# dibbelab/gficf

Measured on AMD Instinct MI355X. Metric: jaccard_edges_per_sec, higher is better.
Workload: dtype int32; 1 GPU; north-star point: 100000 cells x k=30 per GPU; N_total=100000; 8 independent data sets per step, windowed kNN (W=100) with permuted ids; per data set: ingest + edge kernel, one library call, device-resident, one stream, in order (no overlap between data sets or steps); rows taken to hold distinct ids: no duplicate scan in the ingest, the edge kernel's hash-set build reports a repeated id (deferred; cells_total=100000, k=30, partition=cell blocks x1

## Files before the change

### gficf_amd/csrc/jaccard.hip

```cpp
#include <atomic>
#include <cmath>
#include <cstdlib>
#include <cstring>
#include <thread>
#include <type_traits>
#include <vector>

#include "common.h"
#include "halo_map.h"

#include "jaccard_shared.h"
#include "jaccard_ingest.h"
#include "jaccard_edges_general.h"
#include "jaccard_edges_pipe.h"
#include "jaccard_edges_bits.h"
#include "jaccard_sorted.h"
#include "jaccard_direct.h"

namespace {


static_assert(std::is_same<decltype(&k_jaccard_edges<32, false, false, OUT_RMAT, false>), EdgeKernFn>::value &&
              std::is_same<decltype(&k_jaccard_edges<64, false, true, OUT_U16, true>), EdgeKernFn>::value &&
              std::is_same<decltype(&k_jaccard_edges_pipe<32, false, true, OUT_RMAT, true, false, true>), EdgeKernFn>::value &&
// ... 174 lines not shown
      table[(row0 + rr) * pitch + j] = v;
    }
    if (pitch == DUAL_PITCH && compact && kpad == 64) {
      const int lane = threadIdx.x & 63, wave = threadIdx.x >> 6;
      for (int rr = wave; rr < rows_here; rr += 4) {
        const uint32_t* in = s_pk + rr * wpr;
        s_ids[wave][lane] = lane < k ? packed_id(in, lane, bits, wpr, mask) : 0u;
        __builtin_amdgcn_fence(__ATOMIC_ACQ_REL, "wavefront");
        planar_row_build(s_ids[wave], k, ((in[fl_w] >> fl_b) & 1u) != 0u, s_prow[wave], lane);
        if (lane < 32) table[(row0 + rr) * pitch + 32 + lane] = s_prow[wave][lane];
        __builtin_amdgcn_fence(__ATOMIC_ACQ_REL, "wavefront");
      }
    }
    __syncthreads();
  }
}

template <typename T>
int launch_ingest(gficf_ctx* ctx, const T* d_idx, int64_t n_rows, int k, int64_t ld, int64_t N_total,
                  uint32_t* table, int zero_ok = 0) {
  if (sorted_fmt(k)) return launch_ingest_sorted<T>(ctx, d_idx, n_rows, k, ld, N_total, table, zero_ok);
  const TableFmt f = table_fmt(N_total, k);
  const int64_t cap = (int64_t)ctx->num_cus * 8;
  const int64_t tiles2 = gficf_ceil_div(n_rows, INGEST2_ROWS);
  const unsigned grid2 = (unsigned)(tiles2 < cap ? tiles2 : cap);
  const int64_t tiles = gficf_ceil_div(n_rows, INGEST_ROWS);
  const unsigned grid = (unsigned)(tiles < cap ? tiles : cap);
  static const bool use_reg = getenv("GFICF_JACCARD_INGEST_REG") != nullptr;
  const bool scan = !(ctx->jaccard_assume_distinct && zero_ok == 0);
#define LAUNCH_INGEST_REG(KP, CM)                                                                                          \
  do {                                                                                                                     \
    if (use_reg)                                                                                                           \
      hipLaunchKernelGGL((k_ingest_reg<T, KP, CM>), dim3(grid2), dim3(INGEST2_ROWS), 0, ctx->stream, d_idx, n_rows, k, ld, N_total, \
                         table, ctx->d_status, zero_ok);                                                                   \
    else if (scan)                                                                                                         \
      hipLaunchKernelGGL((k_ingest_tile<T, KP, CM>), dim3(grid), dim3(256), 0, ctx->stream, d_idx, n_rows, k, ld, N_total,  \
                         table, ctx->d_status, zero_ok, gficf_halo_map{});                                                 \
    else                                                                                                                   \
      hipLaunchKernelGGL((k_ingest_tile<T, KP, CM, false, false>), dim3(grid), dim3(256), 0, ctx->stream, d_idx, n_rows, k, ld, N_total, \
                         table, ctx->d_status, zero_ok, gficf_halo_map{});                                                 \
  } while (0)
#define LAUNCH_INGEST(KP, CM)                                                                                   \
  hipLaunchKernelGGL((k_ingest<T, KP, CM>), dim3(grid), dim3(256), 0, ctx->stream, d_idx, n_rows, k, ld, N_total, \
                     table, ctx->d_status, zero_ok, scan ? 1 : 0)
  switch (f.kpad) {
    case 16: LAUNCH_INGEST_REG(16, false); break;
    case 32: if (f.compact) LAUNCH_INGEST_REG(32, true); else LAUNCH_INGEST_REG(32, false); break;
    case 64:
      if (f.dual) {
        if (scan)
          hipLaunchKernelGGL((k_ingest_tile<T, 64, true, false, true, true>), dim3(grid), dim3(256), 0, ctx->stream, d_idx, n_rows, k, ld, N_total,
                             table, ctx->d_status, zero_ok, gficf_halo_map{});
        else
          hipLaunchKernelGGL((k_ingest_tile<T, 64, true, false, false, true>), dim3(grid), dim3(256), 0, ctx->stream, d_idx, n_rows, k, ld, N_total,
                             table, ctx->d_status, zero_ok, gficf_halo_map{});
      } else if (f.compact) LAUNCH_INGEST_REG(64, true); else LAUNCH_INGEST_REG(64, false);
      break;
    case 128: if (f.compact) LAUNCH_INGEST(128, true); else LAUNCH_INGEST(128, false); break;
    default: if (f.compact) LAUNCH_INGEST(256, true); else LAUNCH_INGEST(256, false); break;
  }
#undef LAUNCH_INGEST
#undef LAUNCH_INGEST_REG
  GFICF_HIP_CHECK(hipGetLastError());
  return GFICF_OK;
}

template <typename K>
int edge_blocks_per_cu(K kernel, int threads, size_t lds_bytes, std::atomic<int>& cache, int* out) {
  int v = cache.load(std::memory_order_relaxed);
  if (v == 0) {
    int nb = 0;
    GFICF_HIP_CHECK(hipOccupancyMaxActiveBlocksPerMultiprocessor(&nb, kernel, threads, lds_bytes));
    v = nb > 8 ? 8 : nb > 0 ? nb : 1;
    if (const char* e = getenv("GFICF_JACCARD_BLOCKS_PER_CU")) {
      const int t = atoi(e);
      if (t > 0) v = t;
    }
    cache.store(v, std::memory_order_relaxed);
  }
  *out = v;
  return GFICF_OK;
}

template <int KPAD, bool BIG, bool CMP, int OUT, bool MAP>
int launch_edges_m(gficf_ctx* ctx, const uint32_t* table, int64_t N, int k, int64_t cb, int64_t ce, EdgeOut o) {
  using C = JCfg<KPAD, CMP>;
  static std::atomic<int> bpc_general{0}, bpc_pipe{0}, bpc_pipe_nob16{0};
  constexpr size_t lds_bytes = edges_lds_bytes<KPAD, CMP>();
  int blocks_per_cu = 1;
  static const bool no_pipe = getenv("GFICF_JACCARD_NO_PIPE") != nullptr;
  if constexpr (C::EPL == 1 && C::SPQ <= 4) {
    if (!no_pipe) {
      const bool nob16 = CMP && N < 65536;
      int rc;
      if constexpr (!MAP) {
        if (o.dup_status != nullptr) {
          static std::atomic<int> bpc_nf{0}, bpc_nf_nob16{0};
          if (nob16) rc = edge_blocks_per_cu(k_jaccard_edges_pipe<KPAD, BIG, CMP, OUT, !CMP, false, true>, C::WAVES * 64, lds_bytes, bpc_nf_nob16, &blocks_per_cu);
          else rc = edge_blocks_per_cu(k_jaccard_edges_pipe<KPAD, BIG, CMP, OUT, true, false, true>, C::WAVES * 64, lds_bytes, bpc_nf, &blocks_per_cu);
          if (rc) return rc;
          const int64_t cap_n = (int64_t)ctx->num_cus * blocks_per_cu;
          const int64_t need_n = gficf_ceil_div(gficf_ceil_div(ce - cb, 4), C::WAVES);
          unsigned grid_n = (unsigned)(need_n < cap_n ? need_n : cap_n);
          if (o.xcd && grid_n > 8) grid_n = (grid_n + 7u) & ~7u;
          if (nob16)
            hipLaunchKernelGGL((k_jaccard_edges_pipe<KPAD, BIG, CMP, OUT, !CMP, false, true>), dim3(grid_n), dim3(C::WAVES * 64), lds_bytes, ctx->stream,
                               table, N, k, cb, ce, o);
          else
            hipLaunchKernelGGL((k_jaccard_edges_pipe<KPAD, BIG, CMP, OUT, true, false, true>), dim3(grid_n), dim3(C::WAVES * 64), lds_bytes, ctx->stream,
                               table, N, k, cb, ce, o);
          GFICF_HIP_CHECK(hipGetLastError());
          return GFICF_OK;
        }
      }
      if (nob16) rc = edge_blocks_per_cu(k_jaccard_edges_pipe<KPAD, BIG, CMP, OUT, !CMP, MAP>, C::WAVES * 64, lds_bytes, bpc_pipe_nob16, &blocks_per_cu);
      else rc = edge_blocks_per_cu(k_jaccard_edges_pipe<KPAD, BIG, CMP, OUT, true, MAP>, C::WAVES * 64, lds_bytes, bpc_pipe, &blocks_per_cu);
      if (rc) return rc;
      const int64_t cap = (int64_t)ctx->num_cus * blocks_per_cu;
      const int64_t need4 = gficf_ceil_div(gficf_ceil_div(ce - cb, 4), C::WAVES);
      unsigned grid4 = (unsigned)(need4 < cap ? need4 : cap);
      if (o.xcd && grid4 > 8) grid4 = (grid4 + 7u) & ~7u;
      if (nob16)
        hipLaunchKernelGGL((k_jaccard_edges_pipe<KPAD, BIG, CMP, OUT, !CMP, MAP>), dim3(grid4), dim3(C::WAVES * 64), lds_bytes, ctx->stream,
                           table, N, k, cb, ce, o);
      else
        hipLaunchKernelGGL((k_jaccard_edges_pipe<KPAD, BIG, CMP, OUT, true, MAP>), dim3(grid4), dim3(C::WAVES * 64), lds_bytes, ctx->stream, table,
                           N, k, cb, ce, o);
      GFICF_HIP_CHECK(hipGetLastError());
      return GFICF_OK;
    }
  }
  const int rc = edge_blocks_per_cu(k_jaccard_edges<KPAD, BIG, CMP, OUT, MAP>, C::WAVES * 64, lds_bytes, bpc_general, &blocks_per_cu);
  if (rc) return rc;
  const int64_t blocks_needed = gficf_ceil_div(ce - cb, C::WAVES);
  const int64_t cap = (int64_t)ctx->num_cus * blocks_per_cu;
  unsigned grid = (unsigned)(blocks_needed < cap ? blocks_needed : cap);
  if (o.xcd && grid > 8) grid = (grid + 7u) & ~7u;
  hipLaunchKernelGGL((k_jaccard_edges<KPAD, BIG, CMP, OUT, MAP>), dim3(grid), dim3(C::WAVES * 64), lds_bytes, ctx->stream, table,
                     N, k, cb, ce, o);
  GFICF_HIP_CHECK(hipGetLastError());
  return GFICF_OK;
}

template <int KPAD, bool BIG, bool CMP, int OUT>
int launch_edges_o(gficf_ctx* ctx, const uint32_t* table, int64_t N, int k, int64_t cb, int64_t ce, EdgeOut o) {
  if constexpr (OUT != OUT_U16) {
    if (o.l2g) return launch_edges_m<KPAD, BIG, CMP, OUT, true>(ctx, table, N, k, cb, ce, o);
  }
  return launch_edges_m<KPAD, BIG, CMP, OUT, false>(ctx, table, N, k, cb, ce, o);
}

template <int KPAD, bool BIG, bool CMP>
int launch_edges_t(gficf_ctx* ctx, const uint32_t* table, int64_t N, int k, int64_t cb, int64_t ce, EdgeOut o) {
  if (o.u16) return launch_edges_o<KPAD, BIG, CMP, OUT_U16>(ctx, table, N, k, cb, ce, o);
  if (o.u) return launch_edges_o<KPAD, BIG, CMP, OUT_RMAT_U>(ctx, table, N, k, cb, ce, o);
  return launch_edges_o<KPAD, BIG, CMP, OUT_RMAT>(ctx, table, N, k, cb, ce, o);
}

template <int NST, int OUT, bool MAP>
int launch_bits_m(gficf_ctx* ctx, const uint32_t* table, int64_t N, int k, int64_t cb, int64_t ce, EdgeOut o) {
  static std::atomic<int> bpc{0};
  static std::atomic<bool> attr_set[64];
  if (!attr_set[ctx->device & 63]) {
    GFICF_HIP_CHECK(hipFuncSetAttribute((const void*)k_jaccard_edges_bits<NST, OUT, MAP>, hipFuncAttributeMaxDynamicSharedMemorySize, (int)BITS_LDS_BYTES));
    attr_set[ctx->device & 63] = true;
  }
  int blocks_per_cu = 1;
  const int rc = edge_blocks_per_cu(k_jaccard_edges_bits<NST, OUT, MAP>, BITS_WAVES * 64, BITS_LDS_BYTES, bpc, &blocks_per_cu);
  if (rc) return rc;
  const int64_t need = gficf_ceil_div(ce - cb, BITS_WAVES);
  const int64_t cap = (int64_t)ctx->num_cus * blocks_per_cu;
  unsigned grid = (unsigned)(need < cap ? need : cap);
  if (o.xcd && grid > 8) grid = (grid + 7u) & ~7u;
  hipLaunchKernelGGL((k_jaccard_edges_bits<NST, OUT, MAP>), dim3(grid), dim3(BITS_WAVES * 64), BITS_LDS_BYTES, ctx->stream, table, N, k, cb, ce, o);
  GFICF_HIP_CHECK(hipGetLastError());
  return GFICF_OK;
}

template <int NST>
int launch_bits(gficf_ctx* ctx, const uint32_t* table, int64_t N, int k, int64_t cb, int64_t ce, EdgeOut o) {
  if (o.u16) return launch_bits_m<NST, OUT_U16, false>(ctx, table, N, k, cb, ce, o);
  if (o.u) return o.l2g ? launch_bits_m<NST, OUT_RMAT_U, true>(ctx, table, N, k, cb, ce, o) : launch_bits_m<NST, OUT_RMAT_U, false>(ctx, table, N, k, cb, ce, o);
  return o.l2g ? launch_bits_m<NST, OUT_RMAT, true>(ctx, table, N, k, cb, ce, o) : launch_bits_m<NST, OUT_RMAT, false>(ctx, table, N, k, cb, ce, o);
}

template <int KPAD>
int launch_edges(gficf_ctx* ctx, const uint32_t* table, int64_t N, int k, int64_t cb, int64_t ce, EdgeOut o) {
  if constexpr (KPAD == 64) {
    if (table_fmt(N, k).dual) {
      const int nst = (k + 7) / 8;
      return nst <= 5 ? launch_bits<5>(ctx, table, N, k, cb, ce, o) : nst == 6 ? launch_bits<6>(ctx, table, N, k, cb, ce, o)
                                                                                : launch_bits<7>(ctx, table, N, k, cb, ce, o);
    }
  }
  static const bool force_big = getenv("GFICF_JACCARD_FORCE_BIG") != nullptr;
  const bool big = force_big || N >= (1ll << 24) || N * (int64_t)KPAD * 4 >= (1ll << 32);
  if (KPAD >= 32 && table_fmt(N, k).compact)
    return launch_edges_t<KPAD, false, KPAD >= 32>(ctx, table, N, k, cb, ce, o);
  return big ? launch_edges_t<KPAD, true, false>(ctx, table, N, k, cb, ce, o)
             : launch_edges_t<KPAD, false, false>(ctx, table, N, k, cb, ce, o);
}

int launch_edges_k(gficf_ctx* ctx, const uint32_t* t, int64_t N, int k, int64_t cb, int64_t ce, EdgeOut o) {
  if (sorted_fmt(k)) return launch_edges_sorted(ctx, t, N, k, cb, ce, o);
// ... 684 lines not shown
```

### gficf_amd/csrc/jaccard_edges_pipe.h

```cpp

#pragma once

#include "jaccard_shared.h"

namespace {

template <int KPAD, bool BIG, bool CMP, int OUT, bool B16 = true, bool MAP = false, bool NOFLAG = false>
__global__ __launch_bounds__(jc_threads<KPAD>) void k_jaccard_edges_pipe(
    const uint32_t* __restrict__ table, int64_t N, int k, int64_t cell_begin, int64_t cell_end, EdgeOut o) {
  using C = JCfg<KPAD, CMP>;
  using F = CFmt<KPAD>;
  static_assert(C::EPL == 1 && C::SPQ <= 4, "one batch of gathers per cell");
  static_assert(!(BIG && CMP), "compact rows hold 17-bit ids");
  using off_t = typename std::conditional<BIG, uint64_t, uint32_t>::type;
  constexpr int NST = C::SPQ;
  extern __shared__ unsigned char smem[];
  constexpr uint32_t HBYTES = C::NB * 8;
  constexpr uint32_t SETS = 1;
  constexpr uint32_t WBYTES = SETS * HBYTES;
  uint32_t(*const s_rows)[2][KPAD] = reinterpret_cast<uint32_t(*)[2][KPAD]>(smem + C::WAVES * WBYTES);
  double* const s_lut = reinterpret_cast<double*>(smem + C::WAVES * WBYTES + C::WAVES * 2 * KPAD * 4);
  constexpr uint32_t STAGE_OFF = C::WAVES * WBYTES + C::WAVES * 2 * KPAD * 4 + (GFICF_JACCARD_MAX_K + 1) * 8;
  constexpr uint32_t STAGE_WAVE = 4 * 64 * 8;
  constexpr uint32_t DUPF_OFF = edges_dupflag_off<KPAD, CMP>();

  const int tid = threadIdx.x, lane = tid & 63;
  const int wave = __builtin_amdgcn_readfirstlane(tid >> 6);
  unsigned char* const hbase = smem + wave * WBYTES;
  for (int u = tid; u <= k; u += C::WAVES * 64) s_lut[u] = (double)u / (2.0 * (double)k - (double)u);
  for (int b = lane; b < (int)(SETS * C::NB); b += 64) reinterpret_cast<uint2*>(hbase)[b] = make_uint2(EMPTY, EMPTY);
  for (int t = lane; t < 4 * 64; t += 64) reinterpret_cast<uint2*>(smem + STAGE_OFF + (uint32_t)wave * STAGE_WAVE)[t] = make_uint2(0u, 0u);
  if (lane == 0) *reinterpret_cast<uint32_t*>(smem + DUPF_OFF + (uint32_t)wave * 4u) = 0u;
  __syncthreads();

  const uint32_t wave_off = lds_address(smem) + (uint32_t)(tid >> 6) * WBYTES;
  uint32_t bmask_v = (uint32_t)(C::NB - 1) << 3, bit16_v = 0x10000u;
  asm volatile("" : "+v"(bmask_v), "+v"(bit16_v));
  uint32_t* const ovlist = s_rows[wave][0];
  const char* const tbytes = reinterpret_cast<const char*>(table);
  const int grow = lane / C::LPR, gl = lane % C::LPR;
  const uint32_t gcol = (uint32_t)gl * 16u;
  const unsigned long long lt_mask = (1ull << lane) - 1ull;
  const int64_t nwaves = (int64_t)gridDim.x * C::WAVES;
  constexpr uint32_t ROWB = C::ROWB;
  constexpr int ROWW = ROWB / 4;
  const int hi_abs = F::HIW + (gl >> 2);
  const int hi_l = lane - gl + (hi_abs >> 2), hi_c = hi_abs & 3;
  const bool tail = gl >= F::KC / 8;
  const int slot_c = lane < C::NSLOT ? lane : C::NSLOT - 1;
  const bool slot_ok = lane < C::NSLOT;

  const int64_t first = cell_begin + 4 * ((int64_t)xcd_block(blockIdx.x, gridDim.x, o.xcd) * C::WAVES + wave);
  if (first >= cell_end) return;
  const int64_t last_cell = cell_end - 1;
  const int64_t quad_step = 4 * nwaves - 3;
  const uint32_t stage_w = lds_address(smem) + STAGE_OFF + (uint32_t)(tid >> 6) * STAGE_WAVE;
  int qc0, qc1;
  uint32_t qra0, qra1;
  {
    const int e0 = 2 * lane, e1 = e0 + 1;
    qc0 = (e0 >= k) + (e0 >= 2 * k) + (e0 >= 3 * k);
    qc1 = (e1 >= k) + (e1 >= 2 * k) + (e1 >= 3 * k);
    int j0 = e0 - qc0 * k, j1 = e1 - qc1 * k;
    j0 = j0 < 63 ? j0 : 63;
    j1 = j1 < 63 ? j1 : 63;
    qra0 = stage_w + (uint32_t)(qc0 * 64 + j0) * 8u;
    qra1 = stage_w + (uint32_t)(qc1 * 64 + j1) * 8u;
  }

  struct OwnRaw { uint32_t v, hw, last; };
  auto load_own = [&](int64_t row, OwnRaw& r) {
    const uint32_t* const rw = table + row * ROWW;
    if (!CMP) {
      r.v = rw[slot_c];
      r.hw = 0; r.last = 0;
    } else {
      r.last = rw[ROWW - 1];
      r.v = reinterpret_cast<const uint16_t*>(rw)[slot_c];
      r.hw = (KPAD == 32) ? 0u : rw[F::HIW + (slot_c >> 5)];
    }
  };
  auto decode_own = [&](const OwnRaw& r) -> uint32_t {
    uint32_t x;
    if (!CMP) x = r.v;
    else if (B16) x = r.v | ((((KPAD == 32 ? r.last : r.hw) >> (lane & 31)) & 1u) << 16) | (NOFLAG ? 0u : (r.last & ROW_DUP_FLAG));
    else x = r.v | (NOFLAG ? 0u : (r.last & ROW_DUP_FLAG));
    return slot_ok ? x : 0u;
  };
  auto true_id = [&](uint32_t keyraw) -> uint32_t {
    const uint32_t x = keyraw & ID_MASK;
    return CMP ? (unscramble16(x & 0xFFFFu) | (x & 0x10000u)) : x;
  };
  auto issue_gathers = [&](uint32_t asafe, uint4 (&bv)[NST]) {
#pragma unroll
    for (int st = 0; st < NST; ++st) {
      const uint32_t dst = (uint32_t)__shfl((int)asafe, st * C::RPS + grow);
      const off_t off = (off_t)(dst - 1) * ROWB + gcol;
      bv[st] = *reinterpret_cast<const uint4*>(tbytes + off);
    }
  };
  auto piece_words = [&](const uint4& bv, uint32_t (&wd)[4], uint32_t& hb) -> uint32_t {
    hb = 0;
    if (B16) {
      uint32_t hw;
      if (KPAD == 32) hw = (uint32_t)__builtin_amdgcn_update_dpp(0, (int)bv.w, 0xFF, 0xf, 0xf, false);
      else {
        hw = 0;
        { const uint32_t v = (uint32_t)__shfl((int)bv.z, hi_l); hw = hi_c == 2 ? v : hw; }
        { const uint32_t v = (uint32_t)__shfl((int)bv.w, hi_l); hw = hi_c == 3 ? v : hw; }
      }
      hb = (hw >> ((gl & 3) * 8)) & 0xFFu;
    }
    wd[0] = bv.x; wd[1] = bv.y; wd[2] = bv.z; wd[3] = bv.w;
    if (tail) {
      hb &= (1u << (F::KC % 8)) - 1u;
#pragma unroll
      for (int c = (F::KC % 8) / 2; c < 4; ++c) wd[c] = 0u;
    }
    return (gl == C::LPR - 1) ? bv.w : 0u;
  };

  auto process = [&](uint32_t araw, const uint4 (&bv)[NST], int& u_out) -> bool {
    const uint32_t a = araw & ID_MASK;
    bool slow = NOFLAG ? false : __ballot((araw & ROW_DUP_FLAG) != 0) != 0ull;
    int myslot = -1, nov = 0;
    bool dup_here = false;
    {
      bool over = false;
      if (a != 0) {
        const uint32_t key = a;
        const uint32_t bo = (CMP ? (key & ((uint32_t)(C::NB - 1) << 3)) : bucket_off<KPAD, BIG>(key)) + (uint32_t)wave * WBYTES;
        uint32_t old = atomicCAS(reinterpret_cast<uint32_t*>(smem + bo), EMPTY, key);
        if (old == EMPTY) myslot = (int)bo;
        else {
          dup_here |= old == key;
          old = atomicCAS(reinterpret_cast<uint32_t*>(smem + bo + 4), EMPTY, key);
          if (old == EMPTY) myslot = (int)bo + 4;
          else { dup_here |= old == key; over = true; }
        }
      }
      const unsigned long long om = __ballot(over);
      if (om) {
        if (over) ovlist[nov + __popcll(om & lt_mask)] = a;
        nov += __popcll(om);
        if (nov > 1) {
          wave_lds_fence();
          dup_here |= ovlist_repeats(ovlist, nov);
        }
      }
    }
    wave_lds_fence();
    uint32_t dupflags = 0;
    int myu = 0;
#pragma unroll
    for (int st = 0; st < NST; ++st) {
      int c;
      if (!CMP) {
        uint32_t miss = 0;
        uint32_t id[4] = {bv[st].x & ID_MASK, bv[st].y, bv[st].z, bv[st].w};
        if (!NOFLAG) dupflags |= bv[st].x;
        uint2 h[4];
#pragma unroll
        for (int t = 0; t < 4; ++t) h[t] = lds_read_b64(bucket_off<KPAD, BIG>(id[t]) | wave_off);
#pragma unroll
        for (int t = 0; t < 4; t += 2) {
          const uint32_t m0 = min3u_one(h[t].x ^ id[t], h[t].y ^ id[t]);
          const uint32_t m1 = min3u_one(h[t + 1].x ^ id[t + 1], h[t + 1].y ^ id[t + 1]);
          miss += m0 + m1;
        }
        c = 4 - (int)miss;
        if (nov) {
          for (int t = 0; t < nov; ++t) {
            const uint32_t ov = ovlist[t];
#pragma unroll
            for (int tt = 0; tt < 4; ++tt) c += (id[tt] == ov);
          }
        }
      } else {
        uint32_t wd[4], hb;
        const uint32_t fw = piece_words(bv[st], wd, hb);
        if (!NOFLAG) dupflags |= fw;
        c = probe_compact_piece<B16>(wd, hb, bmask_v, bit16_v, wave_off);
        if (nov) {
          for (int t = 0; t < nov; ++t) {
            const uint32_t ov = ovlist[t];
#pragma unroll
            for (int tt = 0; tt < 8; ++tt) c += (piece_key(wd, hb, tt) == ov);
          }
        }
      }
      const int rowcnt = group_sum<C::LPR>(c);
      const int v = __shfl(rowcnt, (lane % C::RPS) * C::LPR);
      myu = (lane / C::RPS == st) ? v : myu;
    }
    if (dup_here) *reinterpret_cast<uint32_t*>(smem + DUPF_OFF + (uint32_t)wave * 4u) = 1u;
    slow |= __ballot(dup_here || (!NOFLAG && (dupflags & ROW_DUP_FLAG) != 0)) != 0ull;
    if (myslot >= 0) *reinterpret_cast<uint32_t*>(smem + myslot) = EMPTY;
    wave_lds_fence();
    u_out = a != 0 ? myu : 0;
    return slow;
  };

  OwnRaw raw;
  load_own(first, raw);
  uint32_t araw_cur = decode_own(raw);
  uint4 bv_cur[NST];
  uint32_t id_cur = true_id(araw_cur);
  uint32_t gid_cur = MAP ? (uint32_t)o.l2g[(id_cur != 0 ? id_cur : (uint32_t)(first + 1)) - 1] : 0u;
  issue_gathers(id_cur != 0 ? id_cur : (uint32_t)(first + 1), bv_cur);
  {
    const int64_t i1 = first + 1;
    load_own(i1 < cell_end ? i1 : last_cell, raw);
  }
  bool any_slow = false;
  int64_t prev_i = first;
  uint32_t prev_a = 0;
  int prev_u = 0;

  typedef uint32_t v2u __attribute__((ext_vector_type(2)));
  typedef uint32_t v4u __attribute__((ext_vector_type(4)));
  typedef double v2d __attribute__((ext_vector_type(2)));
#ifndef GFICF_EDGE_STORE_AUX
#define GFICF_EDGE_STORE_AUX 2
#endif
  constexpr int EDGE_STORE_AUX = GFICF_EDGE_STORE_AUX;
  auto park_prev = [&](int c) {
    reinterpret_cast<uint2*>(smem + STAGE_OFF + (uint32_t)wave * STAGE_WAVE)[c * 64 + lane] = make_uint2(prev_a, (uint32_t)prev_u);
  };
  auto store_quad = [&](int64_t qfirst, int ncells) {
    wave_lds_fence();
    const uint2 p0 = lds_read_b64(qra0), p1 = lds_read_b64(qra1);
    const int64_t pb = (qfirst - cell_begin) * (int64_t)k;
    const int nedges = ncells * k;
    if (OUT != OUT_U16) {
      const uint32_t c1st = (uint32_t)(qfirst + 1) + o.src_off;
      const bool pos0 = p0.y > 0, pos1 = p1.y > 0;
      const v2d vs = {pos0 ? (double)(c1st + (uint32_t)qc0) : 0.0, pos1 ? (double)(c1st + (uint32_t)qc1) : 0.0};
      const v2d vd = {pos0 ? (double)p0.x : 0.0, pos1 ? (double)p1.x : 0.0};
      const v2d vw = {s_lut[p0.y], s_lut[p1.y]};
      const auto rs = __builtin_amdgcn_make_buffer_rsrc(o.src + pb, 0, nedges * 8, 0x00020000);
      const auto rd = __builtin_amdgcn_make_buffer_rsrc(o.dst + pb, 0, nedges * 8, 0x00020000);
      const auto rw = __builtin_amdgcn_make_buffer_rsrc(o.w + pb, 0, nedges * 8, 0x00020000);
      __builtin_amdgcn_raw_buffer_store_b128(__builtin_bit_cast(v4u, vs), rs, lane * 16, 0, EDGE_STORE_AUX);
      __builtin_amdgcn_raw_buffer_store_b128(__builtin_bit_cast(v4u, vd), rd, lane * 16, 0, EDGE_STORE_AUX);
      __builtin_amdgcn_raw_buffer_store_b128(__builtin_bit_cast(v4u, vw), rw, lane * 16, 0, EDGE_STORE_AUX);
    }
    if (OUT == OUT_RMAT_U) {
      const auto ru = __builtin_amdgcn_make_buffer_rsrc(o.u + pb, 0, nedges * 4, 0x00020000);
      __builtin_amdgcn_raw_buffer_store_b64(v2u{p0.y, p1.y}, ru, lane * 8, 0, 2);
    }
    if (OUT == OUT_U16) {
      const auto ru = __builtin_amdgcn_make_buffer_rsrc(o.u16 + pb, 0, nedges * 2, 0x00020000);
      const auto ru_even = __builtin_amdgcn_make_buffer_rsrc(o.u16 + pb, 0, (nedges & ~1) * 2, 0x00020000);
      __builtin_amdgcn_raw_buffer_store_b32(p0.y | (p1.y << 16), ru_even, lane * 4, 0, 0);
      if (nedges & 1) __builtin_amdgcn_raw_buffer_store_b16((uint16_t)p0.y, ru, lane * 4, 0, 0);
    }
  };

  auto body = [&](int64_t i, const uint4 (&cur)[NST], uint4 (&nxt)[NST], auto cq_tag, auto park_tag) {
    constexpr int CQ = decltype(cq_tag)::value;
    constexpr bool PARK = decltype(park_tag)::value;
    const int64_t i1 = i + (CQ == 3 ? quad_step : 1), i2 = i1 + (CQ == 2 ? quad_step : 1);
    const bool valid1 = i1 < cell_end;
    const uint32_t araw_next = valid1 ? decode_own(raw) : 0u;
    const uint32_t a1 = true_id(araw_next);
    load_own(i2 < cell_end ? i2 : last_cell, raw);
    __builtin_amdgcn_sched_barrier(0);
    const uint32_t gid_next = MAP ? (uint32_t)o.l2g[(a1 != 0 ? a1 : (uint32_t)(i + 1)) - 1] : 0u;
    issue_gathers(a1 != 0 ? a1 : (uint32_t)(i + 1), nxt);
    __builtin_amdgcn_sched_barrier(0);
    if (PARK) park_prev((CQ + 3) & 3);
    if (PARK && CQ == 0) store_quad(i - 4 * nwaves, 4);
    __builtin_amdgcn_sched_barrier(0);
    int u;
    const bool slow = process(araw_cur, cur, u);
    any_slow |= slow;
    prev_i = i;
    prev_a = MAP ? gid_cur : id_cur;
    prev_u = u;
    araw_cur = araw_next;
    id_cur = a1;
    gid_cur = gid_next;
  };

  uint4 bv_b[NST];
  using T_ = std::true_type;
  int64_t i = first;
  int cq_last = 0;
  body(i, bv_cur, bv_b, std::integral_constant<int, 0>{}, std::false_type{});
  for (;;) {
    if (i + 1 >= cell_end) break;
    i += 1; cq_last = 1;
    body(i, bv_b, bv_cur, std::integral_constant<int, 1>{}, T_{});
    if (i + 1 >= cell_end) break;
    i += 1; cq_last = 2;
    body(i, bv_cur, bv_b, std::integral_constant<int, 2>{}, T_{});
    if (i + 1 >= cell_end) break;
    i += 1; cq_last = 3;
    body(i, bv_b, bv_cur, std::integral_constant<int, 3>{}, T_{});
    if (i + quad_step >= cell_end) break;
    i += quad_step; cq_last = 0;
    body(i, bv_cur, bv_b, std::integral_constant<int, 0>{}, T_{});
  }
  park_prev(cq_last);
  store_quad(prev_i - cq_last, cq_last + 1);
  if (any_slow) {
    wave_lds_fence();
    if (*reinterpret_cast<const uint32_t*>(smem + DUPF_OFF + (uint32_t)wave * 4u) != 0u && lane == 0) {
      uint32_t* const st = edge_kernel_dup_status();
      if (st != nullptr) atomicOr(st, GFICF_ST_DUP_IDS);
    }
  }
  if (any_slow) {
    __builtin_amdgcn_s_waitcnt(0);
    for (int64_t n = 0;; ++n) {
      const int64_t c = first + (n >> 2) * 4 * nwaves + (n & 3);
      if (c >= cell_end) break;
      const uint32_t* const rw = table + c * ROWW;
      const uint32_t a = lane < k ? row_slot_id(rw, lane, KPAD, CMP) : 0u;
      bool f = row_dup_flag(rw, KPAD, CMP);
      if (a != 0) f |= row_dup_flag(table + (int64_t)(a - 1) * ROWW, KPAD, CMP);
      if (__ballot(f) != 0ull)
        slow_cell<KPAD, CMP, OUT>(table, c, k, (c - cell_begin) * (int64_t)k, s_rows[wave][0], s_rows[wave][1], lane, o.src, o.dst, o.w,
                                  o.u, o.u16, o.set_mode, s_lut, o.l2g, o.src_off);
    }
  }
}

}
```

### gficf_amd/csrc/jaccard_shared.h

```cpp
#pragma once

#include <atomic>
#include <cmath>
#include <cstdlib>
#include <cstring>
#include <thread>
#include <type_traits>
#include <vector>

#include "common.h"
#include "halo_map.h"

namespace {


constexpr uint32_t ROW_DUP_FLAG = 0x80000000u;
constexpr uint32_t ID_MASK = 0x7FFFFFFFu;
constexpr uint32_t EMPTY = 0xFFFFFFFFu;

__host__ __device__ inline int kpad_for(int k) {
  return k <= 16 ? 16 : k <= 32 ? 32 : k <= 64 ? 64 : k <= 128 ? 128 : 256;
}

template <int KPAD>
// ... 143 lines not shown

template <int KPAD, bool CMP>
struct JCfg {
  static constexpr int ROWB = CMP ? KPAD * 2 : KPAD * 4;
  static constexpr int LPR = ROWB / 16;
  static constexpr int RPS = 64 / LPR;
  static constexpr int IPL = CMP ? 8 : 4;
  static constexpr int NSLOT = CMP ? CFmt<KPAD>::KC : KPAD;
  static constexpr int EPL = KPAD > 64 ? KPAD / 64 : 1;
  static constexpr int SPQ = (KPAD < 64 ? KPAD : 64) / RPS;
  static constexpr int NB = 8 * KPAD;
  static constexpr int WAVES = KPAD <= 128 ? 4 : 2;
#ifndef GFICF_JACCARD_U
#define GFICF_JACCARD_U 8
#endif
  static constexpr int U = SPQ < GFICF_JACCARD_U ? SPQ : GFICF_JACCARD_U;
  static constexpr int LOG2NB = KPAD == 16 ? 7 : KPAD == 32 ? 8 : KPAD == 64 ? 9 : KPAD == 128 ? 10 : 11;
};

template <int KPAD, bool CMP>
constexpr uint32_t edges_dupflag_off() {
  using C = JCfg<KPAD, CMP>;
  return (uint32_t)(C::WAVES * C::NB * 8 + C::WAVES * 2 * KPAD * 4 + (GFICF_JACCARD_MAX_K + 1) * (int)sizeof(double) +
                    ((C::EPL == 1 && C::SPQ <= 4) ? C::WAVES * 4 * 64 * 8 : 0));
}
template <int KPAD, bool CMP>
constexpr size_t edges_lds_bytes() { return (size_t)edges_dupflag_off<KPAD, CMP>() + (size_t)JCfg<KPAD, CMP>::WAVES * 4; }

struct EdgeOut;
__device__ inline uint32_t* edge_kernel_dup_status();

extern "C" __device__ uint32_t gficf_mul_u24(uint32_t a, uint32_t b) __asm("llvm.amdgcn.mul.u24.i32");

template <int KPAD, bool BIG>
__device__ inline uint32_t bucket_off(uint32_t id) {
  constexpr uint32_t HMASK = (uint32_t)(JCfg<KPAD, false>::NB - 1) << 3;
  return (BIG ? id * 0x9E3779B1u : gficf_mul_u24(id, 0x9E3779u)) & HMASK;
}

typedef uint32_t gficf_v2u __attribute__((ext_vector_type(2)));
__device__ inline uint32_t lds_address(const void* p) {
  return (uint32_t)(size_t)(__attribute__((address_space(3))) const unsigned char*)p;
}
__device__ inline uint2 lds_read_b64(uint32_t addr) {
  const gficf_v2u v = *(__attribute__((address_space(3))) const gficf_v2u*)(size_t)addr;
  return make_uint2(v.x, v.y);
}

__device__ inline uint32_t min3u_one(uint32_t a, uint32_t b) {
  uint32_t m;
  asm("v_min3_u32 %0, %1, %2, 1" : "=v"(m) : "v"(a), "v"(b));
  return m;
}

template <int TT>
__device__ inline uint32_t bitop3(uint32_t a, uint32_t b, uint32_t c) {
  uint32_t r;
  asm("v_bitop3_b32 %0, %1, %2, %3 bitop3:%4" : "=v"(r) : "v"(a), "v"(b), "v"(c), "n"(TT));
  return r;
}

__device__ inline int add_lane_bit(int c, unsigned long long m) {
  int r;
  asm("v_addc_co_u32_e64 %0, vcc, %1, 0, %2" : "=v"(r) : "v"(c), "s"(m) : "vcc");
  return r;
}

extern "C" __device__ int gficf_writelane(int value, int lane, int old) __asm("llvm.amdgcn.writelane.i32");

__device__ inline void wave_lds_fence() { __builtin_amdgcn_fence(__ATOMIC_ACQ_REL, "wavefront"); }

__device__ inline bool ovlist_repeats(const uint32_t* ovlist, int nov) {
  uint32_t v[6];
#pragma unroll
  for (int t = 0; t < 6; ++t) v[t] = t < nov ? ovlist[t] : 0xFFFFFFF0u + (uint32_t)t;
  bool r = nov > 6;
#pragma unroll
  for (int a = 1; a < 6; ++a)
#pragma unroll
    for (int b = 0; b < a; ++b) r |= v[a] == v[b];
  return r;
}

struct EdgeOut {
  double* src;
  double* dst;
  double* w;
  int32_t* u;
  uint16_t* u16;
  int set_mode;
  const int32_t* l2g = nullptr;
  uint32_t src_off = 0;
  uint32_t* dup_status = nullptr;
  uint32_t xcd = 1;
};

struct EdgeKernArgs { const uint32_t* table; int64_t N; int k; int64_t cell_begin; int64_t cell_end; EdgeOut o; };
using EdgeKernFn = void (*)(const uint32_t*, int64_t, int, int64_t, int64_t, EdgeOut);
constexpr int EDGE_KERNARG_OUT = (int)offsetof(EdgeKernArgs, o);
static_assert(EDGE_KERNARG_OUT == 40 && offsetof(EdgeKernArgs, cell_end) == 32, "kernel argument block of the edge kernels");
__device__ inline uint32_t* edge_kernel_dup_status() {
#if defined(__HIP_DEVICE_COMPILE__)
  typedef const char __attribute__((address_space(4))) * kptr;
  typedef uint32_t* const __attribute__((address_space(4))) * kslot;
  const kptr ka = (kptr)__builtin_amdgcn_kernarg_segment_ptr();
  return *(kslot)(ka + EDGE_KERNARG_OUT + offsetof(EdgeOut, dup_status));
#else
  return nullptr;
#endif
}

__device__ inline uint32_t xcd_block(uint32_t b, uint32_t nb, uint32_t on) {
  return (on && (nb & 7u) == 0) ? (b & 7u) * (nb >> 3) + (b >> 3) : b;
}

constexpr int OUT_RMAT = 0;
constexpr int OUT_RMAT_U = 1;
constexpr int OUT_U16 = 2;

template <int OUT>
__device__ inline void store_edge(const EdgeOut o, int64_t r, int64_t cell, uint32_t dst, int u,
                                  const double* lut) {
  const bool pos = u > 0;
  if (OUT != OUT_U16) {
    __builtin_nontemporal_store(pos ? (double)((uint32_t)(cell + 1) + o.src_off) : 0.0, o.src + r);
    __builtin_nontemporal_store(pos ? (double)dst : 0.0, o.dst + r);
    __builtin_nontemporal_store(lut[u], o.w + r);
  }
  if (OUT == OUT_RMAT_U) __builtin_nontemporal_store(u, o.u + r);
  if (OUT == OUT_U16) o.u16[r] = (uint16_t)u;
}

template <int KPAD, bool CMP, int OUT>
__device__ __noinline__ void slow_cell(const uint32_t* __restrict__ table, int64_t i, int k, int64_t out_base,
                                       uint32_t* sA, uint32_t* sB, int lane, double* o_src, double* o_dst,
                                       double* o_w, int32_t* o_u, uint16_t* o_u16, int set_mode, const double* lut,
                                       const int32_t* l2g, uint32_t src_off, int pitch = 0) {
  const EdgeOut o{o_src, o_dst, o_w, o_u, o_u16, set_mode, nullptr, src_off};
  const int ROWW = pitch ? pitch : (CMP ? CFmt<KPAD>::ROWW : KPAD);
  for (int e = lane; e < KPAD; e += 64) sA[e] = row_slot_id(table + i * ROWW, e, KPAD, CMP);
  wave_lds_fence();
  for (int s = 0; s < k; ++s) {
    const uint32_t dst = sA[s];
    int u = 0;
    if (dst != 0) {
      for (int e = lane; e < KPAD; e += 64) sB[e] = row_slot_id(table + (int64_t)(dst - 1) * ROWW, e, KPAD, CMP);
      wave_lds_fence();
      int cnt = 0;
      for (int e = lane; e < k; e += 64) {
        const uint32_t b = sB[e];
        if (b != 0) {
          int rank = 0, ca = 0;
          for (int t = 0; t < k; ++t) {
            ca += (sA[t] == b);
            rank += (t < e && sB[t] == b);
          }
          cnt += set_mode ? (rank == 0 && ca > 0) : (rank < ca);
        }
      }
#pragma unroll
      for (int d = 32; d >= 1; d >>= 1) cnt += __shfl_xor(cnt, d);
      u = cnt;
      wave_lds_fence();
    }
    if (lane == 0) store_edge<OUT>(o, out_base + s, i, (l2g && dst) ? (uint32_t)l2g[dst - 1] : dst, u, lut);
  }
}

#ifndef GFICF_PROBE_BATCH
#define GFICF_PROBE_BATCH 8
#endif
__device__ inline uint32_t piece_key(const uint32_t (&wd)[4], uint32_t hb, int t) {
  const uint32_t half = (t & 1) ? (wd[t >> 1] >> 16) : (wd[t >> 1] & 0xFFFFu);
  return half | (((hb >> t) & 1u) << 16);
}
template <bool B16 = true>
__device__ inline int probe_compact_piece(const uint32_t (&wd)[4], uint32_t hb, uint32_t bmask, uint32_t bit16, uint32_t base) {
// ... 46 lines not shown
```

Baseline: 64.03 billion edges/s.

## Balance pipe edge kernel work with per-wave quad-then-remainder cell dealing

Replaces the strided quad-per-wave cell assignment in the pipelined edge kernel with a precomputed deal. Each wave gets an equal number of full quads plus a contiguous share of the leftover cells, so the tail is spread evenly. By default the grid is now sized from cells rather than quads, so more waves can be launched. This is meant to remove load imbalance and idle waves at the end of the grid. It adds index arithmetic per cell, and unaligned u16 stores at the last group need a split store path.

```diff
diff --git a/gficf_amd/csrc/jaccard.hip b/gficf_amd/csrc/jaccard.hip
--- a/gficf_amd/csrc/jaccard.hip
+++ b/gficf_amd/csrc/jaccard.hip
@@ -280,6 +280,15 @@
   return GFICF_OK;
 }
 
+inline unsigned edge_pipe_grid(int64_t cb, int64_t ce, int64_t cap, int waves, EdgeOut& o) {
+  static const bool by_quads = getenv("GFICF_JACCARD_GRID_BY_QUADS") != nullptr;
+  const int64_t need = gficf_ceil_div(by_quads ? gficf_ceil_div(ce - cb, 4) : ce - cb, waves);
+  unsigned grid = (unsigned)(need < cap ? need : cap);
+  if (o.xcd && grid > 8) grid = (grid + 7u) & ~7u;
+  if (grid) o.deal = grid_deal(cb, ce, grid * (uint32_t)waves);
+  return grid;
+}
+
 template <int KPAD, bool BIG, bool CMP, int OUT, bool MAP>
 int launch_edges_m(gficf_ctx* ctx, const uint32_t* table, int64_t N, int k, int64_t cb, int64_t ce, EdgeOut o) {
   using C = JCfg<KPAD, CMP>;
@@ -297,10 +306,7 @@
           if (nob16) rc = edge_blocks_per_cu(k_jaccard_edges_pipe<KPAD, BIG, CMP, OUT, !CMP, false, true>, C::WAVES * 64, lds_bytes, bpc_nf_nob16, &blocks_per_cu);
           else rc = edge_blocks_per_cu(k_jaccard_edges_pipe<KPAD, BIG, CMP, OUT, true, false, true>, C::WAVES * 64, lds_bytes, bpc_nf, &blocks_per_cu);
           if (rc) return rc;
-          const int64_t cap_n = (int64_t)ctx->num_cus * blocks_per_cu;
-          const int64_t need_n = gficf_ceil_div(gficf_ceil_div(ce - cb, 4), C::WAVES);
-          unsigned grid_n = (unsigned)(need_n < cap_n ? need_n : cap_n);
-          if (o.xcd && grid_n > 8) grid_n = (grid_n + 7u) & ~7u;
+          const unsigned grid_n = edge_pipe_grid(cb, ce, (int64_t)ctx->num_cus * blocks_per_cu, C::WAVES, o);
           if (nob16)
             hipLaunchKernelGGL((k_jaccard_edges_pipe<KPAD, BIG, CMP, OUT, !CMP, false, true>), dim3(grid_n), dim3(C::WAVES * 64), lds_bytes, ctx->stream,
                                table, N, k, cb, ce, o);
@@ -314,10 +320,7 @@
       if (nob16) rc = edge_blocks_per_cu(k_jaccard_edges_pipe<KPAD, BIG, CMP, OUT, !CMP, MAP>, C::WAVES * 64, lds_bytes, bpc_pipe_nob16, &blocks_per_cu);
       else rc = edge_blocks_per_cu(k_jaccard_edges_pipe<KPAD, BIG, CMP, OUT, true, MAP>, C::WAVES * 64, lds_bytes, bpc_pipe, &blocks_per_cu);
       if (rc) return rc;
-      const int64_t cap = (int64_t)ctx->num_cus * blocks_per_cu;
-      const int64_t need4 = gficf_ceil_div(gficf_ceil_div(ce - cb, 4), C::WAVES);
-      unsigned grid4 = (unsigned)(need4 < cap ? need4 : cap);
-      if (o.xcd && grid4 > 8) grid4 = (grid4 + 7u) & ~7u;
+      const unsigned grid4 = edge_pipe_grid(cb, ce, (int64_t)ctx->num_cus * blocks_per_cu, C::WAVES, o);
       if (nob16)
         hipLaunchKernelGGL((k_jaccard_edges_pipe<KPAD, BIG, CMP, OUT, !CMP, MAP>), dim3(grid4), dim3(C::WAVES * 64), lds_bytes, ctx->stream,
                            table, N, k, cb, ce, o);
diff --git a/gficf_amd/csrc/jaccard_edges_pipe.h b/gficf_amd/csrc/jaccard_edges_pipe.h
--- a/gficf_amd/csrc/jaccard_edges_pipe.h
+++ b/gficf_amd/csrc/jaccard_edges_pipe.h
@@ -41,7 +41,6 @@
   const int grow = lane / C::LPR, gl = lane % C::LPR;
   const uint32_t gcol = (uint32_t)gl * 16u;
   const unsigned long long lt_mask = (1ull << lane) - 1ull;
-  const int64_t nwaves = (int64_t)gridDim.x * C::WAVES;
   constexpr uint32_t ROWB = C::ROWB;
   constexpr int ROWW = ROWB / 4;
   const int hi_abs = F::HIW + (gl >> 2);
@@ -50,10 +49,14 @@
   const int slot_c = lane < C::NSLOT ? lane : C::NSLOT - 1;
   const bool slot_ok = lane < C::NSLOT;
 
-  const int64_t first = cell_begin + 4 * ((int64_t)xcd_block(blockIdx.x, gridDim.x, o.xcd) * C::WAVES + wave);
-  if (first >= cell_end) return;
-  const int64_t last_cell = cell_end - 1;
-  const int64_t quad_step = 4 * nwaves - 3;
+  const WaveDeal deal = wave_deal(o.deal, gridDim.x * (uint32_t)C::WAVES,
+                                  xcd_block(blockIdx.x, gridDim.x, o.xcd) * (uint32_t)C::WAVES + (uint32_t)wave);
+  if (deal.count == 0) return;
+  auto cell_abs = [&](uint32_t rel) -> int64_t { return cell_begin + (int64_t)rel; };
+  const uint32_t first_rel = deal_cell(deal, 0u);
+  const uint32_t last_rel = deal_cell(deal, deal.count - 1u);
+  const int64_t first = cell_abs(first_rel);
+  const uint32_t id_base = (uint32_t)cell_begin + 1u;
   const uint32_t stage_w = lds_address(smem) + STAGE_OFF + (uint32_t)(tid >> 6) * STAGE_WAVE;
   int qc0, qc1;
   uint32_t qra0, qra1;
@@ -206,14 +209,10 @@
   uint32_t araw_cur = decode_own(raw);
   uint4 bv_cur[NST];
   uint32_t id_cur = true_id(araw_cur);
-  uint32_t gid_cur = MAP ? (uint32_t)o.l2g[(id_cur != 0 ? id_cur : (uint32_t)(first + 1)) - 1] : 0u;
-  issue_gathers(id_cur != 0 ? id_cur : (uint32_t)(first + 1), bv_cur);
-  {
-    const int64_t i1 = first + 1;
-    load_own(i1 < cell_end ? i1 : last_cell, raw);
-  }
+  uint32_t gid_cur = MAP ? (uint32_t)o.l2g[(id_cur != 0 ? id_cur : id_base + first_rel) - 1] : 0u;
+  issue_gathers(id_cur != 0 ? id_cur : id_base + first_rel, bv_cur);
+  load_own(cell_abs(1u < deal.count ? first_rel + 1u : last_rel), raw);
   bool any_slow = false;
-  int64_t prev_i = first;
   uint32_t prev_a = 0;
   int prev_u = 0;
 
@@ -227,13 +226,14 @@
   auto park_prev = [&](int c) {
     reinterpret_cast<uint2*>(smem + STAGE_OFF + (uint32_t)wave * STAGE_WAVE)[c * 64 + lane] = make_uint2(prev_a, (uint32_t)prev_u);
   };
-  auto store_quad = [&](int64_t qfirst, int ncells) {
+  auto store_quad = [&](uint32_t qrel, int ncells, auto last_tag) {
+    constexpr bool LAST = decltype(last_tag)::value;
     wave_lds_fence();
     const uint2 p0 = lds_read_b64(qra0), p1 = lds_read_b64(qra1);
-    const int64_t pb = (qfirst - cell_begin) * (int64_t)k;
+    const int64_t pb = (int64_t)qrel * (int64_t)k;
     const int nedges = ncells * k;
     if (OUT != OUT_U16) {
-      const uint32_t c1st = (uint32_t)(qfirst + 1) + o.src_off;
+      const uint32_t c1st = id_base + qrel + o.src_off;
       const bool pos0 = p0.y > 0, pos1 = p1.y > 0;
       const v2d vs = {pos0 ? (double)(c1st + (uint32_t)qc0) : 0.0, pos1 ? (double)(c1st + (uint32_t)qc1) : 0.0};
       const v2d vd = {pos0 ? (double)p0.x : 0.0, pos1 ? (double)p1.x : 0.0};
@@ -252,30 +252,40 @@
     if (OUT == OUT_U16) {
       const auto ru = __builtin_amdgcn_make_buffer_rsrc(o.u16 + pb, 0, nedges * 2, 0x00020000);
       const auto ru_even = __builtin_amdgcn_make_buffer_rsrc(o.u16 + pb, 0, (nedges & ~1) * 2, 0x00020000);
-      __builtin_amdgcn_raw_buffer_store_b32(p0.y | (p1.y << 16), ru_even, lane * 4, 0, 0);
-      if (nedges & 1) __builtin_amdgcn_raw_buffer_store_b16((uint16_t)p0.y, ru, lane * 4, 0, 0);
-    }
-  };
-
-  auto body = [&](int64_t i, const uint4 (&cur)[NST], uint4 (&nxt)[NST], auto cq_tag, auto park_tag) {
+      if (LAST && (pb & 1)) {
+        __builtin_amdgcn_raw_buffer_store_b16((uint16_t)p0.y, ru, lane * 4, 0, 0);
+        __builtin_amdgcn_raw_buffer_store_b16((uint16_t)p1.y, ru, lane * 4 + 2, 0, 0);
+      } else {
+        __builtin_amdgcn_raw_buffer_store_b32(p0.y | (p1.y << 16), ru_even, lane * 4, 0, 0);
+        if (nedges & 1) __builtin_amdgcn_raw_buffer_store_b16((uint16_t)p0.y, ru, lane * 4, 0, 0);
+      }
+    }
+  };
+
+  uint32_t n4 = 0;
+  uint32_t gf = first_rel, gf_prev = first_rel, gf_next = first_rel;
+  auto body = [&](const uint4 (&cur)[NST], uint4 (&nxt)[NST], auto cq_tag, auto park_tag) {
     constexpr int CQ = decltype(cq_tag)::value;
     constexpr bool PARK = decltype(park_tag)::value;
-    const int64_t i1 = i + (CQ == 3 ? quad_step : 1), i2 = i1 + (CQ == 2 ? quad_step : 1);
-    const bool valid1 = i1 < cell_end;
+    const uint32_t n = n4 + (uint32_t)CQ;
+    const uint32_t i_id = id_base + gf + (uint32_t)CQ;
+    const bool valid1 = n + 1u < deal.count;
+    if (CQ == 2) gf_next = deal_next_group(deal, n4, gf);
+    const uint32_t c2 = CQ < 2 ? gf + (uint32_t)CQ + 2u : gf_next + (uint32_t)(CQ - 2);
+    const int64_t i2 = cell_abs(n + 2u < deal.count ? c2 : last_rel);
     const uint32_t araw_next = valid1 ? decode_own(raw) : 0u;
     const uint32_t a1 = true_id(araw_next);
-    load_own(i2 < cell_end ? i2 : last_cell, raw);
+    load_own(i2, raw);
     __builtin_amdgcn_sched_barrier(0);
-    const uint32_t gid_next = MAP ? (uint32_t)o.l2g[(a1 != 0 ? a1 : (uint32_t)(i + 1)) - 1] : 0u;
-    issue_gathers(a1 != 0 ? a1 : (uint32_t)(i + 1), nxt);
+    const uint32_t gid_next = MAP ? (uint32_t)o.l2g[(a1 != 0 ? a1 : i_id) - 1] : 0u;
+    issue_gathers(a1 != 0 ? a1 : i_id, nxt);
     __builtin_amdgcn_sched_barrier(0);
     if (PARK) park_prev((CQ + 3) & 3);
-    if (PARK && CQ == 0) store_quad(i - 4 * nwaves, 4);
+    if (PARK && CQ == 0) store_quad(gf_prev, 4, std::false_type{});
     __builtin_amdgcn_sched_barrier(0);
     int u;
     const bool slow = process(araw_cur, cur, u);
     any_slow |= slow;
-    prev_i = i;
     prev_a = MAP ? gid_cur : id_cur;
     prev_u = u;
     araw_cur = araw_next;
@@ -285,25 +295,24 @@
 
   uint4 bv_b[NST];
   using T_ = std::true_type;
-  int64_t i = first;
   int cq_last = 0;
-  body(i, bv_cur, bv_b, std::integral_constant<int, 0>{}, std::false_type{});
+  body(bv_cur, bv_b, std::integral_constant<int, 0>{}, std::false_type{});
   for (;;) {
-    if (i + 1 >= cell_end) break;
-    i += 1; cq_last = 1;
-    body(i, bv_b, bv_cur, std::integral_constant<int, 1>{}, T_{});
-    if (i + 1 >= cell_end) break;
-    i += 1; cq_last = 2;
-    body(i, bv_cur, bv_b, std::integral_constant<int, 2>{}, T_{});
-    if (i + 1 >= cell_end) break;
-    i += 1; cq_last = 3;
-    body(i, bv_b, bv_cur, std::integral_constant<int, 3>{}, T_{});
-    if (i + quad_step >= cell_end) break;
-    i += quad_step; cq_last = 0;
-    body(i, bv_cur, bv_b, std::integral_constant<int, 0>{}, T_{});
+    if (n4 + 1u >= deal.count) break;
+    cq_last = 1;
+    body(bv_b, bv_cur, std::integral_constant<int, 1>{}, T_{});
+    if (n4 + 2u >= deal.count) break;
+    cq_last = 2;
+    body(bv_cur, bv_b, std::integral_constant<int, 2>{}, T_{});
+    if (n4 + 3u >= deal.count) break;
+    cq_last = 3;
+    body(bv_b, bv_cur, std::integral_constant<int, 3>{}, T_{});
+    if (n4 + 4u >= deal.count) break;
+    n4 += 4u; gf_prev = gf; gf = gf_next; cq_last = 0;
+    body(bv_cur, bv_b, std::integral_constant<int, 0>{}, T_{});
   }
   park_prev(cq_last);
-  store_quad(prev_i - cq_last, cq_last + 1);
+  store_quad(gf, cq_last + 1, T_{});
   if (any_slow) {
     wave_lds_fence();
     if (*reinterpret_cast<const uint32_t*>(smem + DUPF_OFF + (uint32_t)wave * 4u) != 0u && lane == 0) {
@@ -313,9 +322,8 @@
   }
   if (any_slow) {
     __builtin_amdgcn_s_waitcnt(0);
-    for (int64_t n = 0;; ++n) {
-      const int64_t c = first + (n >> 2) * 4 * nwaves + (n & 3);
-      if (c >= cell_end) break;
+    for (uint32_t n = 0; n < deal.count; ++n) {
+      const int64_t c = cell_abs(deal_cell(deal, n));
       const uint32_t* const rw = table + c * ROWW;
       const uint32_t a = lane < k ? row_slot_id(rw, lane, KPAD, CMP) : 0u;
       bool f = row_dup_flag(rw, KPAD, CMP);
diff --git a/gficf_amd/csrc/jaccard_shared.h b/gficf_amd/csrc/jaccard_shared.h
--- a/gficf_amd/csrc/jaccard_shared.h
+++ b/gficf_amd/csrc/jaccard_shared.h
@@ -249,6 +249,45 @@
   return r;
 }
 
+struct GridDeal {
+  uint32_t R;
+  uint32_t q, x;
+};
+struct WaveDeal {
+  uint32_t quad0;
+  uint32_t pitch;
+  uint32_t nquad;
+  uint32_t rem0;
+  uint32_t count;
+};
+__host__ __device__ inline GridDeal grid_deal(int64_t cell_begin, int64_t cell_end, uint32_t W) {
+  const uint32_t C = cell_end > cell_begin ? (uint32_t)(cell_end - cell_begin) : 0u;
+  GridDeal g;
+  g.R = C / (4u * W);
+  const uint32_t rem = C - g.R * 4u * W;
+  g.q = rem / W;
+  g.x = rem - g.q * W;
+  return g;
+}
+__host__ __device__ inline WaveDeal wave_deal(const GridDeal& g, uint32_t W, uint32_t r) {
+  WaveDeal d;
+  d.pitch = 4u * W;
+  d.quad0 = 4u * r;
+  d.nquad = 4u * g.R;
+  d.rem0 = g.R * d.pitch + r * g.q + (r < g.x ? r : g.x);
+  d.count = d.nquad + g.q + (r < g.x ? 1u : 0u);
+  return d;
+}
+__host__ __device__ inline WaveDeal wave_deal(int64_t cell_begin, int64_t cell_end, uint32_t W, uint32_t r) {
+  return wave_deal(grid_deal(cell_begin, cell_end, W), W, r);
+}
+__host__ __device__ inline uint32_t deal_cell(const WaveDeal& d, uint32_t n) {
+  return n < d.nquad ? d.quad0 + (n >> 2) * d.pitch + (n & 3u) : d.rem0 + (n - d.nquad);
+}
+__host__ __device__ inline uint32_t deal_next_group(const WaveDeal& d, uint32_t n4, uint32_t gfirst) {
+  return n4 + 4u < d.nquad ? gfirst + d.pitch : d.rem0;
+}
+
 struct EdgeOut {
   double* src;
   double* dst;
@@ -260,6 +299,7 @@
   uint32_t src_off = 0;
   uint32_t* dup_status = nullptr;
   uint32_t xcd = 1;
+  GridDeal deal = {0, 0, 0};
 };
 
 struct EdgeKernArgs { const uint32_t* table; int64_t N; int k; int64_t cell_begin; int64_t cell_end; EdgeOut o; };
```

After: 64.06 billion edges/s (median of 4 runs). No clear change (+0.0%).
